# robo-alex/gs-dynamics

Measured on AMD Instinct MI355X. Metric: fwd+bwd Mpix/s at 100k Gaussians, 4x800^2 views, higher is better.
Workload: dtype f32

## Files before the change

### gs-dynamics_amd/csrc/gsr_preprocess_bwd.hip

```cpp
#include "gsr_common.h"

namespace gsr_preprocess_bwd {

__constant__ float kC2[5] = {1.0925484305920792f, -1.0925484305920792f, 0.31539156525252005f,
                             -1.0925484305920792f, 0.5462742152960396f};
__constant__ float kC3[7] = {-0.5900435899266435f, 2.890611442640554f, -0.4570457994644658f,
                             0.3731763325901154f, -0.4570457994644658f, 1.445305721320277f,
                             -0.5900435899266435f};
#define SH_C0 0.28209479177387814f
#define SH_C1 0.4886025119029199f

__device__ __forceinline__ float clampf(float v, float lo, float hi) { return v < lo ? lo : (v > hi ? hi : v); }

template <bool NO_DSH = false>
__device__ void sh_backward(int deg, int M, const float* __restrict__ sh, float3 p, const float* __restrict__ campos,
                            uint32_t clamped, float g0, float g1, float g2, float* __restrict__ dsh, float dmean[3]) {
  float dL[3] = {(clamped & 1u) ? 0.f : g0, (clamped & 2u) ? 0.f : g1, (clamped & 4u) ? 0.f : g2};
  const float ox = p.x - campos[0], oy = p.y - campos[1], oz = p.z - campos[2];
  const float len = sqrtf(ox * ox + oy * oy + oz * oz), inv = 1.0f / len;
  const float x = ox * inv, y = oy * inv, z = oz * inv;
  float basis[16];
#pragma unroll
  for (int k = 0; k < 16; ++k) basis[k] = 0.f;
  float dRdx[3] = {0.f, 0.f, 0.f}, dRdy[3] = {0.f, 0.f, 0.f}, dRdz[3] = {0.f, 0.f, 0.f};
// ... 213 lines not shown
    if (r32 < GSR_AA_FLOOR) {
      *c_out = cf;
    } else {
      const real h = (real)0.3f;
      const real A = U0[0] * T0[0] + U0[1] * T0[1] + U0[2] * T0[2];
      const real C = U1[0] * T1[0] + U1[1] * T1[1] + U1[2] * T1[2];
      const real cr = sqrt(fmax((A * C - b * b) / det, (real)GSR_AA_FLOOR));
      *c_out = (float)cr;
      const real k = (real)o_s / (real)cf * (real)ps.gop / (2.0 * cr * det * det);
      aa_a = k * h * (C * C + h * C + b * b);
      aa_c = k * h * (A * A + h * A + b * b);
      aa_b = -2.0 * k * h * b * (A + C + h);
    }
  }
  const real dL_da = AA ? dL_da0 + aa_a : dL_da0;
  const real dL_dc = AA ? dL_dc0 + aa_c : dL_dc0;
  const real dL_db = AA ? dL_db0 + aa_b : dL_db0;
  gcov[0] += (float)(T0[0] * T0[0] * dL_da + T0[0] * T1[0] * dL_db + T1[0] * T1[0] * dL_dc);
  gcov[3] += (float)(T0[1] * T0[1] * dL_da + T0[1] * T1[1] * dL_db + T1[1] * T1[1] * dL_dc);
  gcov[5] += (float)(T0[2] * T0[2] * dL_da + T0[2] * T1[2] * dL_db + T1[2] * T1[2] * dL_dc);
  gcov[1] += (float)(2.0f * T0[0] * T0[1] * dL_da + (T0[0] * T1[1] + T0[1] * T1[0]) * dL_db + 2.0f * T1[0] * T1[1] * dL_dc);
  gcov[2] += (float)(2.0f * T0[0] * T0[2] * dL_da + (T0[0] * T1[2] + T0[2] * T1[0]) * dL_db + 2.0f * T1[0] * T1[2] * dL_dc);
  gcov[4] += (float)(2.0f * T0[1] * T0[2] * dL_da + (T0[1] * T1[2] + T0[2] * T1[1]) * dL_db + 2.0f * T1[1] * T1[2] * dL_dc);
  real dT0[3], dT1[3];
#pragma unroll
  for (int j = 0; j < 3; ++j) {
    dT0[j] = 2.0f * U0[j] * dL_da + U1[j] * dL_db;
    dT1[j] = 2.0f * U1[j] * dL_dc + U0[j] * dL_db;
  }
  const real dJ00 = dT0[0] * view[0] + dT0[1] * view[4] + dT0[2] * view[8];
  const real dJ02 = dT0[0] * view[2] + dT0[1] * view[6] + dT0[2] * view[10];
  const real dJ11 = dT1[0] * view[1] + dT1[1] * view[5] + dT1[2] * view[9];
  const real dJ12 = dT1[0] * view[2] + dT1[1] * view[6] + dT1[2] * view[10];
  const real itz = 1.0f / tz, itz2 = itz * itz, itz3 = itz2 * itz;
  const real dtx = xm * -fx * itz2 * dJ02;
  const real dty = ym * -fy * itz2 * dJ12;
  real dtz = -fx * itz2 * dJ00 - fy * itz2 * dJ11 + (2.0f * fx * tx) * itz3 * dJ02 + (2.0f * fy * ty) * itz3 * dJ12;
  if (DEPTH) dtz += (real)gz;
  const real det_inv = 1.0f / det;
  const real cA = cc * det_inv, cB = -b * det_inv, cC = a * det_inv;
  const real m2x = -(cA * ps.gmx + cB * ps.gmy) * 0.5f * (real)W;
  gm2[0] = (float)m2x;
  const real m2y = -(cC * ps.gmy + cB * ps.gmx) * 0.5f * (real)H;
  gm2[1] = (float)m2y;
  if (gm2_first) {
    gm2_first[0] = (float)(-(cA * sx_first + cB * sy_first) * 0.5f * (real)W);
    gm2_first[1] = (float)(-(cC * sy_first + cB * sx_first) * 0.5f * (real)H);
  }
  const real hx = (real)proj[0] * (real)p.x + (real)proj[4] * (real)p.y + (real)proj[8] * (real)p.z + (real)proj[12];
  const real hy = (real)proj[1] * (real)p.x + (real)proj[5] * (real)p.y + (real)proj[9] * (real)p.z + (real)proj[13];
  const real hw = (real)proj[3] * (real)p.x + (real)proj[7] * (real)p.y + (real)proj[11] * (real)p.z + (real)proj[15];
  const real mw = 1.0f / (hw + 0.0000001f);
  const real mul1 = hx * mw * mw, mul2 = hy * mw * mw;
  gm3[0] += (float)(view[0] * dtx + view[1] * dty + view[2] * dtz + (proj[0] * mw - proj[3] * mul1) * m2x + (proj[1] * mw - proj[3] * mul2) * m2y);
  gm3[1] += (float)(view[4] * dtx + view[5] * dty + view[6] * dtz + (proj[4] * mw - proj[7] * mul1) * m2x + (proj[5] * mw - proj[7] * mul2) * m2y);
  gm3[2] += (float)(view[8] * dtx + view[9] * dty + view[10] * dtz + (proj[8] * mw - proj[11] * mul1) * m2x + (proj[9] * mw - proj[11] * mul2) * m2y);
  if (CAM) {
    ct->dt[0] = dtx; ct->dt[1] = dty; ct->dt[2] = dtz;
#pragma unroll
    for (int j = 0; j < 3; ++j) { ct->dT0[j] = dT0[j]; ct->dT1[j] = dT1[j]; }
    ct->J00 = J00; ct->J02 = J02; ct->J11 = J11; ct->J12 = J12;
    ct->m2x = m2x; ct->m2y = m2y; ct->hx = hx; ct->hy = hy; ct->mw = mw;
  }
}

__device__ __forceinline__ void cov3_to_scale_rot(const Cov3& cv, float mod, const float gcov[6], float gs[3], float gq[4]) {
  const real dS[3][3] = {{(real)gcov[0], 0.5f * (real)gcov[1], 0.5f * (real)gcov[2]},
                          {0.5f * (real)gcov[1], (real)gcov[3], 0.5f * (real)gcov[4]},
                          {0.5f * (real)gcov[2], 0.5f * (real)gcov[4], (real)gcov[5]}};
  real G[3][3];
#pragma unroll
  for (int jj = 0; jj < 3; ++jj) {
    const real dM0 = 2.0f * (dS[0][0] * cv.R[0][jj] + dS[0][1] * cv.R[1][jj] + dS[0][2] * cv.R[2][jj]) * cv.s[jj];
    const real dM1 = 2.0f * (dS[1][0] * cv.R[0][jj] + dS[1][1] * cv.R[1][jj] + dS[1][2] * cv.R[2][jj]) * cv.s[jj];
    const real dM2 = 2.0f * (dS[2][0] * cv.R[0][jj] + dS[2][1] * cv.R[1][jj] + dS[2][2] * cv.R[2][jj]) * cv.s[jj];
    gs[jj] = (float)((real)mod * (cv.R[0][jj] * dM0 + cv.R[1][jj] * dM1 + cv.R[2][jj] * dM2));
    G[0][jj] = dM0 * cv.s[jj]; G[1][jj] = dM1 * cv.s[jj]; G[2][jj] = dM2 * cv.s[jj];
  }
  const real r = cv.q[0], x = cv.q[1], y = cv.q[2], z = cv.q[3];
  gq[0] = (float)(2.0f * (-z * G[0][1] + y * G[0][2] + z * G[1][0] - x * G[1][2] - y * G[2][0] + x * G[2][1]));
  gq[1] = (float)(2.0f * (y * G[0][1] + z * G[0][2] + y * G[1][0] - 2.0f * x * G[1][1] - r * G[1][2] + z * G[2][0] + r * G[2][1] - 2.0f * x * G[2][2]));
  gq[2] = (float)(2.0f * (-2.0f * y * G[0][0] + x * G[0][1] + r * G[0][2] + x * G[1][0] + z * G[1][2] - r * G[2][0] + z * G[2][1] - 2.0f * y * G[2][2]));
  gq[3] = (float)(2.0f * (-2.0f * z * G[0][0] - r * G[0][1] + x * G[0][2] + r * G[1][0] - 2.0f * z * G[1][1] + y * G[1][2] + x * G[2][0] + y * G[2][1]));
}

__device__ __forceinline__ bool gsr_view_used(const GsrBwdView& w, int i) {
  return !w.used || !w.tracked || *w.tracked == 0u || w.used[i] != 0;
}

#define GSR_PBWD_AA 0
#define GSR_PBWD_DEPTH 0
#include "gsr_preprocess_bwd_kernels.inc"
#undef GSR_PBWD_DEPTH
#define GSR_PBWD_DEPTH 1
#include "gsr_preprocess_bwd_kernels.inc"
#undef GSR_PBWD_DEPTH
#undef GSR_PBWD_AA
#define GSR_PBWD_AA 1
#define GSR_PBWD_DEPTH 0
#include "gsr_preprocess_bwd_kernels.inc"
#undef GSR_PBWD_DEPTH
#define GSR_PBWD_DEPTH 1
#include "gsr_preprocess_bwd_kernels.inc"
#undef GSR_PBWD_DEPTH
#undef GSR_PBWD_AA

#include "gsr_camera_bwd.inc"

}
using namespace gsr_preprocess_bwd;

int gsr_launch_preprocess_bwd(const GsrCam& cam, int P, const float* means3D, const float* scales,
                              const float* rotations, const float* colors_precomp, const float* shs,
                              const float* cov3D_precomp, const int32_t* radii, const GeomState& g,
                              const float4* partials, float* dL_dmeans3D, float* dL_dmeans2D, float* dL_dcolors,
                              float* dL_dopacity, float* dL_dscales, float* dL_drotations, float* dL_dcov3D,
                              float* dL_dsh, const uint32_t* bwd_error, hipStream_t st, const float* dL_dz) {
  if (P <= 0) return 0;
  const dim3 grid((P + GSR_BLOCK - 1) / GSR_BLOCK), block(GSR_BLOCK);
#define GSR_PBWD_ARGS                                                                                              \
  P, cam.W, cam.H, cam.tanfovx, cam.tanfovy, cam.scale_modifier, cam.sh_degree, cam.M, cam.view, cam.proj,       \
      cam.campos, means3D, scales, rotations, colors_precomp, shs, cov3D_precomp, radii, g.offsets, g.clamped,  \
      partials, dL_dmeans3D, dL_dmeans2D, dL_dcolors, dL_dopacity, dL_dscales, dL_drotations, dL_dcov3D, dL_dsh, g.used, g.counters + 1, bwd_error
  if (shs && !dL_dsh) { gsr_set_error("gsr_backward: shs given but dL_dsh is NULL"); return -2; }
  if (cam.antialiasing) {
    { GSR_PROF(dL_dz ? "preprocess_bwd_aa_depth" : "preprocess_bwd_aa", st);
      if (dL_dz && shs) hipLaunchKernelGGL(preprocess_bwd_aa_depth_kernel<true>, grid, block, 0, st, GSR_PBWD_ARGS, dL_dz, g.rec);
      else if (dL_dz) hipLaunchKernelGGL(preprocess_bwd_aa_depth_kernel<false>, grid, block, 0, st, GSR_PBWD_ARGS, dL_dz, g.rec);
      else if (shs) hipLaunchKernelGGL(preprocess_bwd_aa_kernel<true>, grid, block, 0, st, GSR_PBWD_ARGS, g.rec);
      else hipLaunchKernelGGL(preprocess_bwd_aa_kernel<false>, grid, block, 0, st, GSR_PBWD_ARGS, g.rec); }
  } else if (dL_dz) {
    { GSR_PROF("preprocess_bwd_depth", st);
      if (shs) hipLaunchKernelGGL(preprocess_bwd_depth_kernel<true>, grid, block, 0, st, GSR_PBWD_ARGS, dL_dz);
      else hipLaunchKernelGGL(preprocess_bwd_depth_kernel<false>, grid, block, 0, st, GSR_PBWD_ARGS, dL_dz); }
  } else if (shs) {
    { GSR_PROF("preprocess_bwd", st);
  hipLaunchKernelGGL(preprocess_bwd_kernel<true>, grid, block, 0, st, GSR_PBWD_ARGS); }
  } else {
    { GSR_PROF("preprocess_bwd", st);
  hipLaunchKernelGGL(preprocess_bwd_kernel<false>, grid, block, 0, st, GSR_PBWD_ARGS); }
  }
#undef GSR_PBWD_ARGS
  GSR_HIP_CHECK(hipGetLastError());
  return 0;
}

int gsr_launch_preprocess_bwd_views(const GsrBwdViews& vw, int P, float scale_modifier, const float* means3D,
                                    const float* scales, const float* rotations, const float* cov3D_precomp,
                                    float* dL_dmeans3D, float* dL_dcolors, float* dL_dopacity, float* dL_dscales,
                                    float* dL_drotations, float* dL_dcov3D, hipStream_t st, const GsrDepthViews* depth, const GsrAaViews* aa) {
  if (P <= 0) return 0;
  int nact = 0;
  for (int v = 0; v < vw.V; ++v) nact += vw.v[v].fused_alias ? 0 : 1;
  if (aa) {
    GSR_PROF("preprocess_bwd_views_aa", st);
    const GsrAaViews& a = *aa;
    if (nact >= 2) {
#define PBW_AA_LAUNCH(K, MAXW, ...) hipLaunchKernelGGL(K<MAXW>, dim3((P + 63) / 64), dim3(64 * nact),                                     \
                           sizeof(float) * (size_t)nact * (PBW_VALUES + 1) * 64, st, vw, P, scale_modifier, means3D, scales, rotations,       \
                           cov3D_precomp, dL_dmeans3D, dL_dcolors, dL_dopacity, dL_dscales, dL_drotations, dL_dcov3D, __VA_ARGS__)
      if (depth) {
        if (nact <= 4) PBW_AA_LAUNCH(preprocess_bwd_views_waves_aa_depth_kernel, 4, *depth, a);
        else if (nact <= 8) PBW_AA_LAUNCH(preprocess_bwd_views_waves_aa_depth_kernel, 8, *depth, a);
        else PBW_AA_LAUNCH(preprocess_bwd_views_waves_aa_depth_kernel, GSR_MAX_BATCH, *depth, a);
      } else if (nact <= 4) PBW_AA_LAUNCH(preprocess_bwd_views_waves_aa_kernel, 4, a);
      else if (nact <= 8) PBW_AA_LAUNCH(preprocess_bwd_views_waves_aa_kernel, 8, a);
      else PBW_AA_LAUNCH(preprocess_bwd_views_waves_aa_kernel, GSR_MAX_BATCH, a);
#undef PBW_AA_LAUNCH
    } else if (depth) {
      hipLaunchKernelGGL(preprocess_bwd_views_aa_depth_kernel, dim3((P + GSR_BLOCK - 1) / GSR_BLOCK), dim3(GSR_BLOCK), 0, st, vw, P,
                         scale_modifier, means3D, scales, rotations, cov3D_precomp, dL_dmeans3D, dL_dcolors, dL_dopacity,
                         dL_dscales, dL_drotations, dL_dcov3D, *depth, a);
    } else {
      hipLaunchKernelGGL(preprocess_bwd_views_aa_kernel, dim3((P + GSR_BLOCK - 1) / GSR_BLOCK), dim3(GSR_BLOCK), 0, st, vw, P,
                         scale_modifier, means3D, scales, rotations, cov3D_precomp, dL_dmeans3D, dL_dcolors, dL_dopacity,
                         dL_dscales, dL_drotations, dL_dcov3D, a);
    }
    GSR_HIP_CHECK(hipGetLastError());
    return 0;
  }
  if (nact >= 2) {
    { GSR_PROF("preprocess_bwd_views", st);
#define PBW_LAUNCH(MAXW) hipLaunchKernelGGL(preprocess_bwd_views_waves_kernel<MAXW>, dim3((P + 63) / 64), dim3(64 * nact),              \
                           sizeof(float) * (size_t)nact * (PBW_VALUES + 1) * 64, st, vw, P, scale_modifier, means3D, scales, rotations,       \
                           cov3D_precomp, dL_dmeans3D, dL_dcolors, dL_dopacity, dL_dscales, dL_drotations, dL_dcov3D)
#define PBW_LAUNCH_DEPTH(MAXW) hipLaunchKernelGGL(preprocess_bwd_views_waves_depth_kernel<MAXW>, dim3((P + 63) / 64), dim3(64 * nact),  \
                           sizeof(float) * (size_t)nact * (PBW_VALUES + 1) * 64, st, vw, P, scale_modifier, means3D, scales, rotations,       \
                           cov3D_precomp, dL_dmeans3D, dL_dcolors, dL_dopacity, dL_dscales, dL_drotations, dL_dcov3D, *depth)
      if (depth) { if (nact <= 4) PBW_LAUNCH_DEPTH(4); else if (nact <= 8) PBW_LAUNCH_DEPTH(8); else PBW_LAUNCH_DEPTH(GSR_MAX_BATCH); }
      else if (nact <= 4) PBW_LAUNCH(4); else if (nact <= 8) PBW_LAUNCH(8); else PBW_LAUNCH(GSR_MAX_BATCH);
#undef PBW_LAUNCH
#undef PBW_LAUNCH_DEPTH
    }
    GSR_HIP_CHECK(hipGetLastError());
    return 0;
  }
  if (depth) {
    GSR_PROF("preprocess_bwd_views", st);
    hipLaunchKernelGGL(preprocess_bwd_views_depth_kernel, dim3((P + GSR_BLOCK - 1) / GSR_BLOCK), dim3(GSR_BLOCK), 0, st, vw, P,
                       scale_modifier, means3D, scales, rotations, cov3D_precomp, dL_dmeans3D, dL_dcolors, dL_dopacity,
                       dL_dscales, dL_drotations, dL_dcov3D, *depth);
  } else { GSR_PROF("preprocess_bwd_views", st);
    hipLaunchKernelGGL(preprocess_bwd_views_kernel, dim3((P + GSR_BLOCK - 1) / GSR_BLOCK), dim3(GSR_BLOCK), 0, st, vw, P,
                       scale_modifier, means3D, scales, rotations, cov3D_precomp, dL_dmeans3D, dL_dcolors, dL_dopacity,
                       dL_dscales, dL_drotations, dL_dcov3D); }
  GSR_HIP_CHECK(hipGetLastError());
  return 0;
}

int gsr_launch_camera_bwd(const GsrCamViews& cv, bool antialiasing, hipStream_t st) {
  if (cv.V <= 0) return 0;
  {
    GSR_PROF("camera_bwd", st);
    const dim3 grid(cv.nblk, cv.V), block(GSR_BLOCK);
    if (cv.shs && antialiasing) hipLaunchKernelGGL((camera_bwd_kernel<true, true>), grid, block, 0, st, cv);
    else if (cv.shs) hipLaunchKernelGGL((camera_bwd_kernel<true, false>), grid, block, 0, st, cv);
    else if (antialiasing) hipLaunchKernelGGL((camera_bwd_kernel<false, true>), grid, block, 0, st, cv);
    else hipLaunchKernelGGL((camera_bwd_kernel<false, false>), grid, block, 0, st, cv);
  }
  GSR_HIP_CHECK(hipGetLastError());
  {
    GSR_PROF("camera_reduce", st);
    hipLaunchKernelGGL(camera_reduce_kernel, dim3(cv.V), dim3(GSR_BLOCK), 0, st, cv);
  }
  GSR_HIP_CHECK(hipGetLastError());
  return 0;
}
```

### gs-dynamics_amd/csrc/gsr_preprocess_bwd_kernels.inc

```
#if GSR_PBWD_DEPTH && GSR_PBWD_AA
#define GSR_PBWD_NAME(k) k##_aa_depth_kernel
#elif GSR_PBWD_DEPTH
#define GSR_PBWD_NAME(k) k##_depth_kernel
#elif GSR_PBWD_AA
#define GSR_PBWD_NAME(k) k##_aa_kernel
#else
#define GSR_PBWD_NAME(k) k##_kernel
#endif
#if GSR_PBWD_DEPTH
#define GSR_PBWD_DZ_PARAM(...) , __VA_ARGS__
#define GSR_PBWD_DZ(x) (x)
#else
#define GSR_PBWD_DZ_PARAM(...)
#define GSR_PBWD_DZ(x) ((const float*)nullptr)
#endif
#if GSR_PBWD_AA
#define GSR_PBWD_AA_PARAM(...) , __VA_ARGS__
#define GSR_PBWD_AA_ARGS(recs) , cv32, (recs)[GSR_REC_F4 * (size_t)i + 1].y, &caa
#else
#define GSR_PBWD_AA_PARAM(...)
#define GSR_PBWD_AA_ARGS(recs)
#endif

template <bool USE_SH>
__global__ __launch_bounds__(GSR_BLOCK) void GSR_PBWD_NAME(preprocess_bwd)(
    int P, int W, int H, float tanfovx, float tanfovy, float mod, int sh_degree, int M,
    const float* __restrict__ view, const float* __restrict__ proj, const float* __restrict__ campos,
    const float* __restrict__ means3D, const float* __restrict__ scales, const float* __restrict__ rotations,
    const float* __restrict__ colors_precomp, const float* __restrict__ shs, const float* __restrict__ cov3D_precomp,
    const int32_t* __restrict__ radii, const uint32_t* __restrict__ offsets, const uint32_t* __restrict__ clamped,
    const float4* __restrict__ partials, float* __restrict__ dL_dmeans3D, float* __restrict__ dL_dmeans2D,
    float* __restrict__ dL_dcolors, float* __restrict__ dL_dopacity, float* __restrict__ dL_dscales,
    float* __restrict__ dL_drot, float* __restrict__ dL_dcov3D, float* __restrict__ dL_dsh,
    const uint8_t* __restrict__ used, const uint32_t* __restrict__ tracked, const uint32_t* __restrict__ bwd_error GSR_PBWD_DZ_PARAM(const float* __restrict__ dL_dz)
    GSR_PBWD_AA_PARAM(const float4* __restrict__ rec)) {
  const int i = blockIdx.x * GSR_BLOCK + threadIdx.x;
  if (i >= P) return;
  float gm3[3] = {0.f, 0.f, 0.f}, gm2[2] = {0.f, 0.f}, gcol[3] = {0.f, 0.f, 0.f}, gop = 0.f;
  float gs[3] = {0.f, 0.f, 0.f}, gq[4] = {0.f, 0.f, 0.f, 0.f}, gcov[6] = {0.f, 0.f, 0.f, 0.f, 0.f, 0.f};
  const bool alive = radii[i] > 0 && (!used || !tracked || *tracked == 0u || used[i] != 0);
  if (USE_SH && !alive && dL_dsh) {
    for (int k = 0; k < M * 3; ++k) dL_dsh[(size_t)i * M * 3 + k] = 0.f;
  }
  if (alive) {
    const PartialSum ps = reduce_partials(partials, offsets[i], offsets[i + 1], USE_SH || dL_dcolors != nullptr);
    gop = ps.gop;
    const float3 p = make_float3(means3D[3 * i], means3D[3 * i + 1], means3D[3 * i + 2]);
    if (USE_SH) {
      float dmean_sh[3] = {0.f, 0.f, 0.f};
      sh_backward(sh_degree, M, shs + (size_t)i * M * 3, p, campos, clamped[i], ps.dr, ps.dg, ps.db,
                  dL_dsh + (size_t)i * M * 3, dmean_sh);
      gm3[0] = dmean_sh[0]; gm3[1] = dmean_sh[1]; gm3[2] = dmean_sh[2];
    } else {
      gcol[0] = ps.dr; gcol[1] = ps.dg; gcol[2] = ps.db;
    }
    Cov3 cv;
    build_cov3(i, mod, scales, rotations, cov3D_precomp, cv);
#if GSR_PBWD_AA
    float cv32[6], caa = 1.f;
    build_cov3_f32(i, mod, scales, rotations, cov3D_precomp, cv32);
#endif
    if (GSR_PBWD_DEPTH) view_chain<true, GSR_PBWD_AA>(view, proj, W, H, tanfovx, tanfovy, p, cv.c, ps, gcov, gm3, gm2, 0.f, 0.f, nullptr,
                                                      reduce_partials_dz(GSR_PBWD_DZ(dL_dz), offsets[i], offsets[i + 1]) GSR_PBWD_AA_ARGS(rec));
    else view_chain<false, GSR_PBWD_AA>(view, proj, W, H, tanfovx, tanfovy, p, cv.c, ps, gcov, gm3, gm2, 0.f, 0.f, nullptr, 0.f GSR_PBWD_AA_ARGS(rec));
#if GSR_PBWD_AA
    gop = caa * ps.gop;
#endif
    if (!cov3D_precomp) cov3_to_scale_rot(cv, mod, gcov, gs, gq);
  }
  if (bwd_error && *bwd_error != 0u) gm3[0] = gm3[1] = gm3[2] = __builtin_nanf("");
  dL_dmeans3D[3 * i] = gm3[0]; dL_dmeans3D[3 * i + 1] = gm3[1]; dL_dmeans3D[3 * i + 2] = gm3[2];
  dL_dmeans2D[3 * i] = gm2[0]; dL_dmeans2D[3 * i + 1] = gm2[1]; dL_dmeans2D[3 * i + 2] = 0.f;
  if (dL_dcolors) { dL_dcolors[3 * i] = gcol[0]; dL_dcolors[3 * i + 1] = gcol[1]; dL_dcolors[3 * i + 2] = gcol[2]; }
  dL_dopacity[i] = gop;
  if (dL_dscales) { dL_dscales[3 * i] = gs[0]; dL_dscales[3 * i + 1] = gs[1]; dL_dscales[3 * i + 2] = gs[2]; }
  if (dL_drot) { dL_drot[4 * i] = gq[0]; dL_drot[4 * i + 1] = gq[1]; dL_drot[4 * i + 2] = gq[2]; dL_drot[4 * i + 3] = gq[3]; }
  if (dL_dcov3D) {
#pragma unroll
    for (int k = 0; k < 6; ++k) dL_dcov3D[6 * i + k] = gcov[k];
  }
}

__global__ __launch_bounds__(GSR_BLOCK) void GSR_PBWD_NAME(preprocess_bwd_views)(
    GsrBwdViews vw, int P, float mod, const float* __restrict__ means3D, const float* __restrict__ scales,
    const float* __restrict__ rotations, const float* __restrict__ cov3D_precomp, float* __restrict__ dL_dmeans3D,
    float* __restrict__ dL_dcolors, float* __restrict__ dL_dopacity, float* __restrict__ dL_dscales,
    float* __restrict__ dL_drot, float* __restrict__ dL_dcov3D GSR_PBWD_DZ_PARAM(GsrDepthViews dz) GSR_PBWD_AA_PARAM(GsrAaViews aa)) {
  const int i = blockIdx.x * GSR_BLOCK + threadIdx.x;
  if (i >= P) return;
  float gm3[3] = {0.f, 0.f, 0.f}, gcol[3] = {0.f, 0.f, 0.f}, gop = 0.f;
  float gs[3] = {0.f, 0.f, 0.f}, gq[4] = {0.f, 0.f, 0.f, 0.f}, gcov[6] = {0.f, 0.f, 0.f, 0.f, 0.f, 0.f};
  const float3 p = make_float3(means3D[3 * i], means3D[3 * i + 1], means3D[3 * i + 2]);
  Cov3 cv;
  build_cov3(i, mod, scales, rotations, cov3D_precomp, cv);
#if GSR_PBWD_AA
  float cv32[6];
  build_cov3_f32(i, mod, scales, rotations, cov3D_precomp, cv32);
#endif
  bool any = false;
  for (int v = 0; v < vw.V; ++v) {
    const GsrBwdView& w = vw.v[v];
    if (w.fused_alias) continue;
    float gm2[2] = {0.f, 0.f}, gm2a[2] = {0.f, 0.f};
    const bool pair = w.partner_dL_dmeans2D != nullptr;
    if (w.radii[i] > 0 && gsr_view_used(w, i)) {
      any = true;
      const PartialSum ps = reduce_partials(w.partials, min(w.offsets[i], w.cap), min(w.offsets[i + 1], w.cap),
                                            pair || w.dL_dcolors != nullptr || dL_dcolors != nullptr);
#if GSR_PBWD_AA
      float caa = 1.f;
#else
      gop += ps.gop;
#endif
      if (pair) {
        view_chain<false, GSR_PBWD_AA>(w.view, w.proj, w.W, w.H, w.tanfovx, w.tanfovy, p, cv.c, ps, gcov, gm3, gm2, ps.dr, ps.dg, gm2a,
                                       0.f GSR_PBWD_AA_ARGS(aa.rec[v]));
      } else {
        if (w.dL_dcolors) { w.dL_dcolors[3 * i] = ps.dr; w.dL_dcolors[3 * i + 1] = ps.dg; w.dL_dcolors[3 * i + 2] = ps.db; }
        else { gcol[0] += ps.dr; gcol[1] += ps.dg; gcol[2] += ps.db; }
        if (GSR_PBWD_DEPTH && GSR_PBWD_DZ(dz.dL_dz[v]))
          view_chain<true, GSR_PBWD_AA>(w.view, w.proj, w.W, w.H, w.tanfovx, w.tanfovy, p, cv.c, ps, gcov, gm3, gm2, 0.f, 0.f, nullptr,
                                        reduce_partials_dz(GSR_PBWD_DZ(dz.dL_dz[v]), min(w.offsets[i], w.cap), min(w.offsets[i + 1], w.cap))
                                        GSR_PBWD_AA_ARGS(aa.rec[v]));
        else view_chain<false, GSR_PBWD_AA>(w.view, w.proj, w.W, w.H, w.tanfovx, w.tanfovy, p, cv.c, ps, gcov, gm3, gm2, 0.f, 0.f, nullptr,
                                            0.f GSR_PBWD_AA_ARGS(aa.rec[v]));
      }
#if GSR_PBWD_AA
      gop += caa * ps.gop;
#endif
    } else if (w.dL_dcolors) {
      w.dL_dcolors[3 * i] = 0.f; w.dL_dcolors[3 * i + 1] = 0.f; w.dL_dcolors[3 * i + 2] = 0.f;
    }
    if (pair) {
      w.dL_dmeans2D[3 * i] = gm2a[0]; w.dL_dmeans2D[3 * i + 1] = gm2a[1]; w.dL_dmeans2D[3 * i + 2] = 0.f;
      float* m2b = w.partner_dL_dmeans2D;
      m2b[3 * i] = gm2[0] - gm2a[0]; m2b[3 * i + 1] = gm2[1] - gm2a[1]; m2b[3 * i + 2] = 0.f;
    } else {
      w.dL_dmeans2D[3 * i] = gm2[0]; w.dL_dmeans2D[3 * i + 1] = gm2[1]; w.dL_dmeans2D[3 * i + 2] = 0.f;
    }
  }
  if (any && !cov3D_precomp) cov3_to_scale_rot(cv, mod, gcov, gs, gq);
  if (vw.bwd_error && *vw.bwd_error != 0u) gm3[0] = gm3[1] = gm3[2] = __builtin_nanf("");
  dL_dmeans3D[3 * i] = gm3[0]; dL_dmeans3D[3 * i + 1] = gm3[1]; dL_dmeans3D[3 * i + 2] = gm3[2];
  if (dL_dcolors) { dL_dcolors[3 * i] = gcol[0]; dL_dcolors[3 * i + 1] = gcol[1]; dL_dcolors[3 * i + 2] = gcol[2]; }
  if (vw.d_raw_rot) {
    reinterpret_cast<float4*>(vw.d_raw_rot)[i] =
        gsr_act_rotation_bwd(reinterpret_cast<const float4*>(vw.raw_rot)[i], make_float4(gq[0], gq[1], gq[2], gq[3]));
    const float o = vw.act_op[i];
    vw.d_raw_op[i] = gop * o * (1.0f - o);
#pragma unroll
    for (int k = 0; k < 3; ++k) vw.d_raw_sc[3 * (size_t)i + k] = gs[k] * vw.act_sc[3 * (size_t)i + k];
  }
  if (dL_dopacity) dL_dopacity[i] = gop;
  if (dL_dscales) { dL_dscales[3 * i] = gs[0]; dL_dscales[3 * i + 1] = gs[1]; dL_dscales[3 * i + 2] = gs[2]; }
  if (dL_drot) { dL_drot[4 * i] = gq[0]; dL_drot[4 * i + 1] = gq[1]; dL_drot[4 * i + 2] = gq[2]; dL_drot[4 * i + 3] = gq[3]; }
  if (dL_dcov3D) {
#pragma unroll
    for (int k = 0; k < 6; ++k) dL_dcov3D[6 * i + k] = gcov[k];
  }
}

#ifndef PBW_VALUES
#define PBW_VALUES 13
#endif
template <int MAXW>
__global__ __launch_bounds__(64 * MAXW) void GSR_PBWD_NAME(preprocess_bwd_views_waves)(
    GsrBwdViews vw, int P, float mod, const float* __restrict__ means3D, const float* __restrict__ scales,
    const float* __restrict__ rotations, const float* __restrict__ cov3D_precomp, float* __restrict__ dL_dmeans3D,
    float* __restrict__ dL_dcolors, float* __restrict__ dL_dopacity, float* __restrict__ dL_dscales,
    float* __restrict__ dL_drot, float* __restrict__ dL_dcov3D GSR_PBWD_DZ_PARAM(GsrDepthViews dz) GSR_PBWD_AA_PARAM(GsrAaViews aa)) {
  extern __shared__ float s_part[];
  const int lane = threadIdx.x & 63, wv = __builtin_amdgcn_readfirstlane((int)(threadIdx.x >> 6)), nw = (int)(blockDim.x >> 6);
  const int i = blockIdx.x * 64 + lane;
  const bool live = i < P;
  int v = -1;
  for (int u = 0, k = 0; u < vw.V; ++u)
    if (!vw.v[u].fused_alias) { if (k == wv) { v = u; break; } ++k; }
  const GsrBwdView& w = vw.v[v < 0 ? 0 : v];
  float3 p = make_float3(0.f, 0.f, 0.f);
  Cov3 cv;
#if GSR_PBWD_AA
  float cv32[6];
#endif
  if (live) {
    p = make_float3(means3D[3 * i], means3D[3 * i + 1], means3D[3 * i + 2]);
    build_cov3(i, mod, scales, rotations, cov3D_precomp, cv);
#if GSR_PBWD_AA
    build_cov3_f32(i, mod, scales, rotations, cov3D_precomp, cv32);
#endif
  }
  float gm3[3] = {0.f, 0.f, 0.f}, gcol[3] = {0.f, 0.f, 0.f}, gop = 0.f, gcov[6] = {0.f, 0.f, 0.f, 0.f, 0.f, 0.f};
  float seen = 0.f;
  if (live && v >= 0) {
    float gm2[2] = {0.f, 0.f}, gm2a[2] = {0.f, 0.f};
    const bool pair = w.partner_dL_dmeans2D != nullptr;
    if (w.radii[i] > 0 && gsr_view_used(w, i)) {
      seen = 1.f;
      const PartialSum ps = reduce_partials(w.partials, min(w.offsets[i], w.cap), min(w.offsets[i + 1], w.cap),
                                            pair || w.dL_dcolors != nullptr || dL_dcolors != nullptr);
      gop = ps.gop;
#if GSR_PBWD_AA
      float caa = 1.f;
#endif
      if (pair) {
        view_chain<false, GSR_PBWD_AA>(w.view, w.proj, w.W, w.H, w.tanfovx, w.tanfovy, p, cv.c, ps, gcov, gm3, gm2, ps.dr, ps.dg, gm2a,
                                       0.f GSR_PBWD_AA_ARGS(aa.rec[v]));
      } else {
        if (w.dL_dcolors) { w.dL_dcolors[3 * i] = ps.dr; w.dL_dcolors[3 * i + 1] = ps.dg; w.dL_dcolors[3 * i + 2] = ps.db; }
        else { gcol[0] = ps.dr; gcol[1] = ps.dg; gcol[2] = ps.db; }
        if (GSR_PBWD_DEPTH && GSR_PBWD_DZ(dz.dL_dz[v]))
          view_chain<true, GSR_PBWD_AA>(w.view, w.proj, w.W, w.H, w.tanfovx, w.tanfovy, p, cv.c, ps, gcov, gm3, gm2, 0.f, 0.f, nullptr,
                                        reduce_partials_dz(GSR_PBWD_DZ(dz.dL_dz[v]), min(w.offsets[i], w.cap), min(w.offsets[i + 1], w.cap))
                                        GSR_PBWD_AA_ARGS(aa.rec[v]));
        else view_chain<false, GSR_PBWD_AA>(w.view, w.proj, w.W, w.H, w.tanfovx, w.tanfovy, p, cv.c, ps, gcov, gm3, gm2, 0.f, 0.f, nullptr,
                                            0.f GSR_PBWD_AA_ARGS(aa.rec[v]));
      }
#if GSR_PBWD_AA
      gop = caa * ps.gop;
#endif
    } else if (w.dL_dcolors) {
      w.dL_dcolors[3 * i] = 0.f; w.dL_dcolors[3 * i + 1] = 0.f; w.dL_dcolors[3 * i + 2] = 0.f;
    }
    if (pair) {
      w.dL_dmeans2D[3 * i] = gm2a[0]; w.dL_dmeans2D[3 * i + 1] = gm2a[1]; w.dL_dmeans2D[3 * i + 2] = 0.f;
      float* m2b = w.partner_dL_dmeans2D;
      m2b[3 * i] = gm2[0] - gm2a[0]; m2b[3 * i + 1] = gm2[1] - gm2a[1]; m2b[3 * i + 2] = 0.f;
    } else {
      w.dL_dmeans2D[3 * i] = gm2[0]; w.dL_dmeans2D[3 * i + 1] = gm2[1]; w.dL_dmeans2D[3 * i + 2] = 0.f;
    }
  }
  float* mine = s_part + (size_t)wv * (PBW_VALUES + 1) * 64 + lane;
#pragma unroll
  for (int k = 0; k < 6; ++k) mine[k * 64] = gcov[k];
#pragma unroll
  for (int k = 0; k < 3; ++k) { mine[(6 + k) * 64] = gm3[k]; mine[(10 + k) * 64] = gcol[k]; }
  mine[9 * 64] = gop;
  mine[PBW_VALUES * 64] = seen;
  __syncthreads();
  if (wv != 0 || !live) return;
  bool any = seen != 0.f;
  for (int u = 1; u < nw; ++u) {
    const float* q = s_part + (size_t)u * (PBW_VALUES + 1) * 64 + lane;
#pragma unroll
    for (int k = 0; k < 6; ++k) gcov[k] += q[k * 64];
#pragma unroll
    for (int k = 0; k < 3; ++k) { gm3[k] += q[(6 + k) * 64]; gcol[k] += q[(10 + k) * 64]; }
    gop += q[9 * 64];
    any = any || q[PBW_VALUES * 64] != 0.f;
  }
  float gs[3] = {0.f, 0.f, 0.f}, gq[4] = {0.f, 0.f, 0.f, 0.f};
  if (any && !cov3D_precomp) cov3_to_scale_rot(cv, mod, gcov, gs, gq);
  if (vw.bwd_error && *vw.bwd_error != 0u) gm3[0] = gm3[1] = gm3[2] = __builtin_nanf("");
  dL_dmeans3D[3 * i] = gm3[0]; dL_dmeans3D[3 * i + 1] = gm3[1]; dL_dmeans3D[3 * i + 2] = gm3[2];
  if (dL_dcolors) { dL_dcolors[3 * i] = gcol[0]; dL_dcolors[3 * i + 1] = gcol[1]; dL_dcolors[3 * i + 2] = gcol[2]; }
  if (vw.d_raw_rot) {
    reinterpret_cast<float4*>(vw.d_raw_rot)[i] =
        gsr_act_rotation_bwd(reinterpret_cast<const float4*>(vw.raw_rot)[i], make_float4(gq[0], gq[1], gq[2], gq[3]));
    const float o = vw.act_op[i];
    vw.d_raw_op[i] = gop * o * (1.0f - o);
#pragma unroll
    for (int k = 0; k < 3; ++k) vw.d_raw_sc[3 * (size_t)i + k] = gs[k] * vw.act_sc[3 * (size_t)i + k];
  }
  if (dL_dopacity) dL_dopacity[i] = gop;
  if (dL_dscales) { dL_dscales[3 * i] = gs[0]; dL_dscales[3 * i + 1] = gs[1]; dL_dscales[3 * i + 2] = gs[2]; }
  if (dL_drot) { dL_drot[4 * i] = gq[0]; dL_drot[4 * i + 1] = gq[1]; dL_drot[4 * i + 2] = gq[2]; dL_drot[4 * i + 3] = gq[3]; }
  if (dL_dcov3D) {
#pragma unroll
    for (int k = 0; k < 6; ++k) dL_dcov3D[6 * i + k] = gcov[k];
  }
}

#undef GSR_PBWD_NAME
#undef GSR_PBWD_DZ_PARAM
#undef GSR_PBWD_DZ
#undef GSR_PBWD_AA_PARAM
#undef GSR_PBWD_AA_ARGS
```

Baseline: 5698.

## Compute covariance once per Gaussian in wave 0 and share via LDS across view waves

The multi-view preprocess backward kernel used to rebuild the 3D covariance in every wave, one wave per active view. Now only wave 0 loads scale and rotation, builds the covariance once and publishes it through shared memory. The block is also capped at a fixed number of waves that loop over the views in rounds, keeping a running sum in LDS. This removes duplicated covariance math and global loads and fixes the launch-bounds template, at the cost of extra barriers, more LDS, and recomputing the covariance in wave 0 before the scale/rotation backward pass.

New measurement: 5660. No clear change (-0.7%).

```diff
diff --git a/gs-dynamics_amd/csrc/gsr_preprocess_bwd.hip b/gs-dynamics_amd/csrc/gsr_preprocess_bwd.hip
--- a/gs-dynamics_amd/csrc/gsr_preprocess_bwd.hip
+++ b/gs-dynamics_amd/csrc/gsr_preprocess_bwd.hip
@@ -389,21 +389,16 @@
   if (P <= 0) return 0;
   int nact = 0;
   for (int v = 0; v < vw.V; ++v) nact += vw.v[v].fused_alias ? 0 : 1;
+  const int nwaves = nact < PBW_WAVES ? nact : PBW_WAVES;
+  const size_t lds = 64 * 6 * (sizeof(double) + (aa ? sizeof(float) : 0)) + sizeof(float) * (size_t)nwaves * (PBW_VALUES + 1) * 64;
+#define PBW_LAUNCH(K, ...) hipLaunchKernelGGL(K, dim3((P + 63) / 64), dim3(64 * nwaves), lds, st, vw, P, scale_modifier, means3D, scales, \
+                           rotations, cov3D_precomp, dL_dmeans3D, dL_dcolors, dL_dopacity, dL_dscales, dL_drotations, dL_dcov3D, ##__VA_ARGS__)
   if (aa) {
     GSR_PROF("preprocess_bwd_views_aa", st);
     const GsrAaViews& a = *aa;
     if (nact >= 2) {
-#define PBW_AA_LAUNCH(K, MAXW, ...) hipLaunchKernelGGL(K<MAXW>, dim3((P + 63) / 64), dim3(64 * nact),                                     \
-                           sizeof(float) * (size_t)nact * (PBW_VALUES + 1) * 64, st, vw, P, scale_modifier, means3D, scales, rotations,       \
-                           cov3D_precomp, dL_dmeans3D, dL_dcolors, dL_dopacity, dL_dscales, dL_drotations, dL_dcov3D, __VA_ARGS__)
-      if (depth) {
-        if (nact <= 4) PBW_AA_LAUNCH(preprocess_bwd_views_waves_aa_depth_kernel, 4, *depth, a);
-        else if (nact <= 8) PBW_AA_LAUNCH(preprocess_bwd_views_waves_aa_depth_kernel, 8, *depth, a);
-        else PBW_AA_LAUNCH(preprocess_bwd_views_waves_aa_depth_kernel, GSR_MAX_BATCH, *depth, a);
-      } else if (nact <= 4) PBW_AA_LAUNCH(preprocess_bwd_views_waves_aa_kernel, 4, a);
-      else if (nact <= 8) PBW_AA_LAUNCH(preprocess_bwd_views_waves_aa_kernel, 8, a);
-      else PBW_AA_LAUNCH(preprocess_bwd_views_waves_aa_kernel, GSR_MAX_BATCH, a);
-#undef PBW_AA_LAUNCH
+      if (depth) PBW_LAUNCH(preprocess_bwd_views_waves_aa_depth_kernel, *depth, a);
+      else PBW_LAUNCH(preprocess_bwd_views_waves_aa_kernel, a);
     } else if (depth) {
       hipLaunchKernelGGL(preprocess_bwd_views_aa_depth_kernel, dim3((P + GSR_BLOCK - 1) / GSR_BLOCK), dim3(GSR_BLOCK), 0, st, vw, P,
                          scale_modifier, means3D, scales, rotations, cov3D_precomp, dL_dmeans3D, dL_dcolors, dL_dopacity,
@@ -418,20 +413,13 @@
   }
   if (nact >= 2) {
     { GSR_PROF("preprocess_bwd_views", st);
-#define PBW_LAUNCH(MAXW) hipLaunchKernelGGL(preprocess_bwd_views_waves_kernel<MAXW>, dim3((P + 63) / 64), dim3(64 * nact),              \
-                           sizeof(float) * (size_t)nact * (PBW_VALUES + 1) * 64, st, vw, P, scale_modifier, means3D, scales, rotations,       \
-                           cov3D_precomp, dL_dmeans3D, dL_dcolors, dL_dopacity, dL_dscales, dL_drotations, dL_dcov3D)
-#define PBW_LAUNCH_DEPTH(MAXW) hipLaunchKernelGGL(preprocess_bwd_views_waves_depth_kernel<MAXW>, dim3((P + 63) / 64), dim3(64 * nact),  \
-                           sizeof(float) * (size_t)nact * (PBW_VALUES + 1) * 64, st, vw, P, scale_modifier, means3D, scales, rotations,       \
-                           cov3D_precomp, dL_dmeans3D, dL_dcolors, dL_dopacity, dL_dscales, dL_drotations, dL_dcov3D, *depth)
-      if (depth) { if (nact <= 4) PBW_LAUNCH_DEPTH(4); else if (nact <= 8) PBW_LAUNCH_DEPTH(8); else PBW_LAUNCH_DEPTH(GSR_MAX_BATCH); }
-      else if (nact <= 4) PBW_LAUNCH(4); else if (nact <= 8) PBW_LAUNCH(8); else PBW_LAUNCH(GSR_MAX_BATCH);
-#undef PBW_LAUNCH
-#undef PBW_LAUNCH_DEPTH
+      if (depth) PBW_LAUNCH(preprocess_bwd_views_waves_depth_kernel, *depth);
+      else PBW_LAUNCH(preprocess_bwd_views_waves_kernel);
     }
     GSR_HIP_CHECK(hipGetLastError());
     return 0;
   }
+#undef PBW_LAUNCH
   if (depth) {
     GSR_PROF("preprocess_bwd_views", st);
     hipLaunchKernelGGL(preprocess_bwd_views_depth_kernel, dim3((P + GSR_BLOCK - 1) / GSR_BLOCK), dim3(GSR_BLOCK), 0, st, vw, P,
diff --git a/gs-dynamics_amd/csrc/gsr_preprocess_bwd_kernels.inc b/gs-dynamics_amd/csrc/gsr_preprocess_bwd_kernels.inc
--- a/gs-dynamics_amd/csrc/gsr_preprocess_bwd_kernels.inc
+++ b/gs-dynamics_amd/csrc/gsr_preprocess_bwd_kernels.inc
@@ -162,94 +162,162 @@
 
 #ifndef PBW_VALUES
 #define PBW_VALUES 13
-#endif
-template <int MAXW>
-__global__ __launch_bounds__(64 * MAXW) void GSR_PBWD_NAME(preprocess_bwd_views_waves)(
+#define PBW_WAVES 4
+#endif
+#if GSR_PBWD_AA
+#define PBW_COV_BYTES (64 * 6 * (sizeof(double) + sizeof(float)))
+#else
+#define PBW_COV_BYTES (64 * 6 * sizeof(double))
+#endif
+__global__ __launch_bounds__(64 * PBW_WAVES) void GSR_PBWD_NAME(preprocess_bwd_views_waves)(
     GsrBwdViews vw, int P, float mod, const float* __restrict__ means3D, const float* __restrict__ scales,
     const float* __restrict__ rotations, const float* __restrict__ cov3D_precomp, float* __restrict__ dL_dmeans3D,
     float* __restrict__ dL_dcolors, float* __restrict__ dL_dopacity, float* __restrict__ dL_dscales,
     float* __restrict__ dL_drot, float* __restrict__ dL_dcov3D GSR_PBWD_DZ_PARAM(GsrDepthViews dz) GSR_PBWD_AA_PARAM(GsrAaViews aa)) {
-  extern __shared__ float s_part[];
+  extern __shared__ double s_cov[];
+  float* const s_part = reinterpret_cast<float*>(reinterpret_cast<char*>(s_cov) + PBW_COV_BYTES);
   const int lane = threadIdx.x & 63, wv = __builtin_amdgcn_readfirstlane((int)(threadIdx.x >> 6)), nw = (int)(blockDim.x >> 6);
   const int i = blockIdx.x * 64 + lane;
   const bool live = i < P;
-  int v = -1;
-  for (int u = 0, k = 0; u < vw.V; ++u)
-    if (!vw.v[u].fused_alias) { if (k == wv) { v = u; break; } ++k; }
-  const GsrBwdView& w = vw.v[v < 0 ? 0 : v];
+  int nact = 0;
+  for (int u = 0; u < vw.V; ++u) nact += vw.v[u].fused_alias ? 0 : 1;
   float3 p = make_float3(0.f, 0.f, 0.f);
-  Cov3 cv;
+  real c3[6];
 #if GSR_PBWD_AA
   float cv32[6];
-#endif
+  float* const s_cov32 = reinterpret_cast<float*>(s_cov + 6 * 64);
+#endif
+  float rot4[4] = {0.f, 0.f, 0.f, 0.f}, sc3[3] = {0.f, 0.f, 0.f};
   if (live) {
     p = make_float3(means3D[3 * i], means3D[3 * i + 1], means3D[3 * i + 2]);
-    build_cov3(i, mod, scales, rotations, cov3D_precomp, cv);
-#if GSR_PBWD_AA
-    build_cov3_f32(i, mod, scales, rotations, cov3D_precomp, cv32);
-#endif
-  }
-  float gm3[3] = {0.f, 0.f, 0.f}, gcol[3] = {0.f, 0.f, 0.f}, gop = 0.f, gcov[6] = {0.f, 0.f, 0.f, 0.f, 0.f, 0.f};
-  float seen = 0.f;
-  if (live && v >= 0) {
-    float gm2[2] = {0.f, 0.f}, gm2a[2] = {0.f, 0.f};
+    if (wv == 0) {
+      if (!cov3D_precomp) {
+#pragma unroll
+        for (int k = 0; k < 4; ++k) rot4[k] = rotations[4 * i + k];
+#pragma unroll
+        for (int k = 0; k < 3; ++k) sc3[k] = scales[3 * i + k];
+      }
+      Cov3 cv;
+      build_cov3(0, mod, sc3, rot4, cov3D_precomp ? cov3D_precomp + 6 * (size_t)i : nullptr, cv);
+#pragma unroll
+      for (int k = 0; k < 6; ++k) s_cov[k * 64 + lane] = c3[k] = cv.c[k];
+#if GSR_PBWD_AA
+      build_cov3_f32(0, mod, sc3, rot4, cov3D_precomp ? cov3D_precomp + 6 * (size_t)i : nullptr, cv32);
+#pragma unroll
+      for (int k = 0; k < 6; ++k) s_cov32[k * 64 + lane] = cv32[k];
+#endif
+    }
+  }
+  bool any = false;
+  float gm3[3], gcol[3], gop, gcov[6];
+  for (int r0 = 0; r0 < nact; r0 += nw) {
+    int v = -1;
+    for (int u = 0, k = 0; u < vw.V; ++u)
+      if (!vw.v[u].fused_alias) { if (k == r0 + wv) { v = u; break; } ++k; }
+    const GsrBwdView& w = vw.v[v < 0 ? 0 : v];
+#pragma unroll
+    for (int k = 0; k < 6; ++k) gcov[k] = 0.f;
+#pragma unroll
+    for (int k = 0; k < 3; ++k) gm3[k] = gcol[k] = 0.f;
+    gop = 0.f;
+    float seen = 0.f;
     const bool pair = w.partner_dL_dmeans2D != nullptr;
-    if (w.radii[i] > 0 && gsr_view_used(w, i)) {
-      seen = 1.f;
-      const PartialSum ps = reduce_partials(w.partials, min(w.offsets[i], w.cap), min(w.offsets[i + 1], w.cap),
-                                            pair || w.dL_dcolors != nullptr || dL_dcolors != nullptr);
-      gop = ps.gop;
-#if GSR_PBWD_AA
-      float caa = 1.f;
-#endif
+    const bool mine_used = live && v >= 0 && w.radii[i] > 0 && gsr_view_used(w, i);
+    PartialSum ps = {0.f, 0.f, 0.f, 0.f, 0.f, 0.f, 0.f, 0.f, 0.f};
+    if (mine_used) ps = reduce_partials(w.partials, min(w.offsets[i], w.cap), min(w.offsets[i + 1], w.cap),
+                                        pair || w.dL_dcolors != nullptr || dL_dcolors != nullptr);
+    if (r0 == 0) {
+      __syncthreads();
+      if (live && wv != 0) {
+#pragma unroll
+        for (int k = 0; k < 6; ++k) c3[k] = s_cov[k * 64 + lane];
+#if GSR_PBWD_AA
+#pragma unroll
+        for (int k = 0; k < 6; ++k) cv32[k] = s_cov32[k * 64 + lane];
+#endif
+      }
+    }
+    if (live && v >= 0) {
+      float gm2[2] = {0.f, 0.f}, gm2a[2] = {0.f, 0.f};
+      if (mine_used) {
+        seen = 1.f;
+        gop = ps.gop;
+#if GSR_PBWD_AA
+        float caa = 1.f;
+#endif
+        if (pair) {
+          view_chain<false, GSR_PBWD_AA>(w.view, w.proj, w.W, w.H, w.tanfovx, w.tanfovy, p, c3, ps, gcov, gm3, gm2, ps.dr, ps.dg, gm2a,
+                                         0.f GSR_PBWD_AA_ARGS(aa.rec[v]));
+        } else {
+          if (w.dL_dcolors) { w.dL_dcolors[3 * i] = ps.dr; w.dL_dcolors[3 * i + 1] = ps.dg; w.dL_dcolors[3 * i + 2] = ps.db; }
+          else { gcol[0] = ps.dr; gcol[1] = ps.dg; gcol[2] = ps.db; }
+          if (GSR_PBWD_DEPTH && GSR_PBWD_DZ(dz.dL_dz[v]))
+            view_chain<true, GSR_PBWD_AA>(w.view, w.proj, w.W, w.H, w.tanfovx, w.tanfovy, p, c3, ps, gcov, gm3, gm2, 0.f, 0.f, nullptr,
+                                          reduce_partials_dz(GSR_PBWD_DZ(dz.dL_dz[v]), min(w.offsets[i], w.cap), min(w.offsets[i + 1], w.cap))
+                                          GSR_PBWD_AA_ARGS(aa.rec[v]));
+          else view_chain<false, GSR_PBWD_AA>(w.view, w.proj, w.W, w.H, w.tanfovx, w.tanfovy, p, c3, ps, gcov, gm3, gm2, 0.f, 0.f, nullptr,
+                                              0.f GSR_PBWD_AA_ARGS(aa.rec[v]));
+        }
+#if GSR_PBWD_AA
+        gop = caa * ps.gop;
+#endif
+      } else if (w.dL_dcolors) {
+        w.dL_dcolors[3 * i] = 0.f; w.dL_dcolors[3 * i + 1] = 0.f; w.dL_dcolors[3 * i + 2] = 0.f;
+      }
       if (pair) {
-        view_chain<false, GSR_PBWD_AA>(w.view, w.proj, w.W, w.H, w.tanfovx, w.tanfovy, p, cv.c, ps, gcov, gm3, gm2, ps.dr, ps.dg, gm2a,
-                                       0.f GSR_PBWD_AA_ARGS(aa.rec[v]));
+        w.dL_dmeans2D[3 * i] = gm2a[0]; w.dL_dmeans2D[3 * i + 1] = gm2a[1]; w.dL_dmeans2D[3 * i + 2] = 0.f;
+        float* m2b = w.partner_dL_dmeans2D;
+        m2b[3 * i] = gm2[0] - gm2a[0]; m2b[3 * i + 1] = gm2[1] - gm2a[1]; m2b[3 * i + 2] = 0.f;
       } else {
-        if (w.dL_dcolors) { w.dL_dcolors[3 * i] = ps.dr; w.dL_dcolors[3 * i + 1] = ps.dg; w.dL_dcolors[3 * i + 2] = ps.db; }
-        else { gcol[0] = ps.dr; gcol[1] = ps.dg; gcol[2] = ps.db; }
-        if (GSR_PBWD_DEPTH && GSR_PBWD_DZ(dz.dL_dz[v]))
-          view_chain<true, GSR_PBWD_AA>(w.view, w.proj, w.W, w.H, w.tanfovx, w.tanfovy, p, cv.c, ps, gcov, gm3, gm2, 0.f, 0.f, nullptr,
-                                        reduce_partials_dz(GSR_PBWD_DZ(dz.dL_dz[v]), min(w.offsets[i], w.cap), min(w.offsets[i + 1], w.cap))
-                                        GSR_PBWD_AA_ARGS(aa.rec[v]));
-        else view_chain<false, GSR_PBWD_AA>(w.view, w.proj, w.W, w.H, w.tanfovx, w.tanfovy, p, cv.c, ps, gcov, gm3, gm2, 0.f, 0.f, nullptr,
-                                            0.f GSR_PBWD_AA_ARGS(aa.rec[v]));
-      }
-#if GSR_PBWD_AA
-      gop = caa * ps.gop;
-#endif
-    } else if (w.dL_dcolors) {
-      w.dL_dcolors[3 * i] = 0.f; w.dL_dcolors[3 * i + 1] = 0.f; w.dL_dcolors[3 * i + 2] = 0.f;
-    }
-    if (pair) {
-      w.dL_dmeans2D[3 * i] = gm2a[0]; w.dL_dmeans2D[3 * i + 1] = gm2a[1]; w.dL_dmeans2D[3 * i + 2] = 0.f;
-      float* m2b = w.partner_dL_dmeans2D;
-      m2b[3 * i] = gm2[0] - gm2a[0]; m2b[3 * i + 1] = gm2[1] - gm2a[1]; m2b[3 * i + 2] = 0.f;
-    } else {
-      w.dL_dmeans2D[3 * i] = gm2[0]; w.dL_dmeans2D[3 * i + 1] = gm2[1]; w.dL_dmeans2D[3 * i + 2] = 0.f;
-    }
-  }
-  float* mine = s_part + (size_t)wv * (PBW_VALUES + 1) * 64 + lane;
-#pragma unroll
-  for (int k = 0; k < 6; ++k) mine[k * 64] = gcov[k];
-#pragma unroll
-  for (int k = 0; k < 3; ++k) { mine[(6 + k) * 64] = gm3[k]; mine[(10 + k) * 64] = gcol[k]; }
-  mine[9 * 64] = gop;
-  mine[PBW_VALUES * 64] = seen;
-  __syncthreads();
+        w.dL_dmeans2D[3 * i] = gm2[0]; w.dL_dmeans2D[3 * i + 1] = gm2[1]; w.dL_dmeans2D[3 * i + 2] = 0.f;
+      }
+    }
+    if (wv != 0) {
+      float* mine = s_part + (size_t)wv * (PBW_VALUES + 1) * 64 + lane;
+#pragma unroll
+      for (int k = 0; k < 6; ++k) mine[k * 64] = gcov[k];
+#pragma unroll
+      for (int k = 0; k < 3; ++k) { mine[(6 + k) * 64] = gm3[k]; mine[(10 + k) * 64] = gcol[k]; }
+      mine[9 * 64] = gop;
+      mine[PBW_VALUES * 64] = seen;
+    }
+    __syncthreads();
+    if (wv == 0) {
+      float* const run = s_part + lane;
+      if (r0 != 0) {
+#pragma unroll
+        for (int k = 0; k < 6; ++k) gcov[k] = run[k * 64] + gcov[k];
+#pragma unroll
+        for (int k = 0; k < 3; ++k) { gm3[k] = run[(6 + k) * 64] + gm3[k]; gcol[k] = run[(10 + k) * 64] + gcol[k]; }
+        gop = run[9 * 64] + gop;
+      }
+      any = any || seen != 0.f;
+      for (int u = 1; u < nw; ++u) {
+        const float* q = s_part + (size_t)u * (PBW_VALUES + 1) * 64 + lane;
+#pragma unroll
+        for (int k = 0; k < 6; ++k) gcov[k] += q[k * 64];
+#pragma unroll
+        for (int k = 0; k < 3; ++k) { gm3[k] += q[(6 + k) * 64]; gcol[k] += q[(10 + k) * 64]; }
+        gop += q[9 * 64];
+        any = any || q[PBW_VALUES * 64] != 0.f;
+      }
+      if (r0 + nw < nact) {
+#pragma unroll
+        for (int k = 0; k < 6; ++k) run[k * 64] = gcov[k];
+#pragma unroll
+        for (int k = 0; k < 3; ++k) { run[(6 + k) * 64] = gm3[k]; run[(10 + k) * 64] = gcol[k]; }
+        run[9 * 64] = gop;
+      }
+    }
+    if (r0 + nw < nact) __syncthreads();
+  }
   if (wv != 0 || !live) return;
-  bool any = seen != 0.f;
-  for (int u = 1; u < nw; ++u) {
-    const float* q = s_part + (size_t)u * (PBW_VALUES + 1) * 64 + lane;
-#pragma unroll
-    for (int k = 0; k < 6; ++k) gcov[k] += q[k * 64];
-#pragma unroll
-    for (int k = 0; k < 3; ++k) { gm3[k] += q[(6 + k) * 64]; gcol[k] += q[(10 + k) * 64]; }
-    gop += q[9 * 64];
-    any = any || q[PBW_VALUES * 64] != 0.f;
-  }
   float gs[3] = {0.f, 0.f, 0.f}, gq[4] = {0.f, 0.f, 0.f, 0.f};
-  if (any && !cov3D_precomp) cov3_to_scale_rot(cv, mod, gcov, gs, gq);
+  if (any && !cov3D_precomp) {
+    Cov3 cv;
+    build_cov3(0, mod, sc3, rot4, nullptr, cv);
+    cov3_to_scale_rot(cv, mod, gcov, gs, gq);
+  }
   if (vw.bwd_error && *vw.bwd_error != 0u) gm3[0] = gm3[1] = gm3[2] = __builtin_nanf("");
   dL_dmeans3D[3 * i] = gm3[0]; dL_dmeans3D[3 * i + 1] = gm3[1]; dL_dmeans3D[3 * i + 2] = gm3[2];
   if (dL_dcolors) { dL_dcolors[3 * i] = gcol[0]; dL_dcolors[3 * i + 1] = gcol[1]; dL_dcolors[3 * i + 2] = gcol[2]; }
@@ -270,6 +338,7 @@
   }
 }
 
+#undef PBW_COV_BYTES
 #undef GSR_PBWD_NAME
 #undef GSR_PBWD_DZ_PARAM
 #undef GSR_PBWD_DZ
```
